# Zhongxu-Wang/ArtSpeech

Measured on AMD Instinct MI355X. Metric: mel frames/sec (whole job; per-GPU = value / n_gpus), acoustic-model inference path, batch 32 x 200-frame utterances, higher is better.
Workload: dtype f32 (f16x3 split-operand MFMA, fp32 accumulate)

## Files before the change

### artspeech_amd/csrc/lstm.hip

```cpp
#include "common.h"
#include "artspeech_hip.h"
#define AS_FILE_CLS AS_CLS_LSTM

#define NB 2

static __device__ __forceinline__ float sigmoidf_(float x) { return __builtin_amdgcn_rcpf(1.0f + __expf(-x)); }
static __device__ __forceinline__ float tanhf_(float x)
{
    const float e = __expf(-2.0f * fabsf(x));
    const float t = (1.0f - e) * __builtin_amdgcn_rcpf(1.0f + e);
    return x < 0.f ? -t : t;
}

template <int CTRL>
static __device__ __forceinline__ float quad_dpp(float v)
{
    return __int_as_float(__builtin_amdgcn_mov_dpp(__float_as_int(v), CTRL, 0xf, 0xf, true));
}

struct LstmJobs { BiLstmJob j[AS_MAX_LSTM_JOBS]; };

static __device__ __forceinline__ void lds_barrier()
{
    asm volatile("s_waitcnt lgkmcnt(0)\n\ts_barrier" ::: "memory");
}

template <int HREG>
__global__ void __launch_bounds__(HREG ? 4 * HREG : 1024)
bilstm_kernel(const LstmJobs jobs, const int* __restrict__ col_off, int B, int Hrt)
{
    extern __shared__ __attribute__((aligned(16))) float sm[];
    const int H = HREG ? HREG : Hrt;
    float* hs = sm;
    float* gs = sm + 2 * H * NB;
    __shared__ int s_off[NB], s_len[NB];

    const BiLstmJob job = jobs.j[blockIdx.z];
    const int dir = blockIdx.y;
    const int u0 = blockIdx.x * NB;
    const int r = threadIdx.x;
    const int G = 4 * H;
    if (r < NB) {
        const int u = u0 + r;
        s_off[r] = u < B ? col_off[u] : 0;
        s_len[r] = u < B ? col_off[u + 1] - col_off[u] : 0;
    }
    for (int i = r; i < 2 * H * NB; i += G) hs[i] = 0.f;
    __syncthreads();
    int Lmax = 0;
#pragma unroll
    for (int u = 0; u < NB; ++u) Lmax = s_len[u] > Lmax ? s_len[u] : Lmax;

    const float* w = job.whh_t + (size_t)dir * H * G + r;
    float wreg[HREG ? HREG : 1];
    if (HREG) {
#pragma unroll
        for (int k = 0; k < HREG; ++k) wreg[k] = w[(size_t)k * G];
    }
    const int unit = r % H, q = r / H;
    float c = 0.f;

    auto load_gx = [&](int t, float (&g)[NB]) {
#pragma unroll
        for (int u = 0; u < NB; ++u) {
            const int L = s_len[u];
            const int pos = dir ? L - 1 - t : t;
            g[u] = (t < L) ? job.gx_tm[(size_t)(s_off[u] + pos) * job.ldg + dir * G + r] : 0.f;
        }
    };
    float gnext[NB];
    load_gx(0, gnext);

    for (int t = 0; t < Lmax; ++t) {
        const float* hc = hs + (t & 1) * H * NB;
        float* hn = hs + ((t + 1) & 1) * H * NB;
        float acc[NB];
#pragma unroll
        for (int u = 0; u < NB; ++u) acc[u] = gnext[u];
        if (t + 1 < Lmax) load_gx(t + 1, gnext);
        if (HREG) {
#pragma unroll
            for (int k = 0; k < HREG; ++k) {
                const float2 h2 = *reinterpret_cast<const float2*>(hc + k * NB);
                acc[0] += wreg[k] * h2.x; acc[1] += wreg[k] * h2.y;
            }
        } else {
            for (int k0 = 0; k0 < H; k0 += 8) {
                float wk[8];
#pragma unroll
                for (int i = 0; i < 8; ++i) wk[i] = w[(size_t)(k0 + i) * G];
#pragma unroll
                for (int i = 0; i < 8; ++i) {
                    const float2 h2 = *reinterpret_cast<const float2*>(hc + (k0 + i) * NB);
                    acc[0] += wk[i] * h2.x; acc[1] += wk[i] * h2.y;
                }
            }
        }
        *reinterpret_cast<float2*>(gs + r * NB) = make_float2(acc[0], acc[1]);
        lds_barrier();
        if (q < NB) {
            const int u = q;
            const int L = s_len[u];
            if (t < L) {
                const float ig = sigmoidf_(gs[(unit)*NB + u]);
                const float fg = sigmoidf_(gs[(H + unit) * NB + u]);
                const float gg = tanhf_(gs[(2 * H + unit) * NB + u]);
                const float og = sigmoidf_(gs[(3 * H + unit) * NB + u]);
                c = fg * c + ig * gg;
                const float hv = og * tanhf_(c);
                hn[unit * NB + u] = hv;
                const int pos = dir ? L - 1 - t : t;
                job.out[(size_t)(dir * H + unit) * job.ldo + s_off[u] + pos] = hv;
            }
        }
        lds_barrier();
    }
}

template <int H, int KREG, int KLDS>
__global__ void __launch_bounds__(2 * H)
bilstm_big_kernel(const LstmJobs jobs, const int* __restrict__ col_off, int B)
{
    constexpr int G = 4 * H, NT = 2 * H, KS = H - KREG - KLDS, SB = 4;
    static_assert(KS >= 0 && KS % SB == 0, "split of the k range");
    extern __shared__ __attribute__((aligned(16))) float sm[];
    float* hs = sm;
    float* gs = hs + 2 * H * NB;
    float* wl = gs + G * NB;
    __shared__ int s_off[NB], s_len[NB];

    const BiLstmJob job = jobs.j[blockIdx.z];
    const int dir = blockIdx.y;
    const int u0 = blockIdx.x * NB;
    const int tid = threadIdx.x;
    if (tid < NB) {
        const int u = u0 + tid;
        s_off[tid] = u < B ? col_off[u] : 0;
        s_len[tid] = u < B ? col_off[u + 1] - col_off[u] : 0;
    }
    for (int i = tid; i < 2 * H * NB; i += NT) hs[i] = 0.f;
    const float* w = job.whh_t + (size_t)dir * H * G + tid;
    float wa[KREG], wb[KREG];
#pragma unroll
    for (int k = 0; k < KREG; ++k) {
        wa[k] = w[(size_t)k * G];
        wb[k] = w[(size_t)k * G + NT];
    }
#pragma unroll 4
    for (int k = 0; k < KLDS; ++k) {
        wl[k * G + tid] = w[(size_t)(KREG + k) * G];
        wl[k * G + NT + tid] = w[(size_t)(KREG + k) * G + NT];
    }
    const float* ws = w + (size_t)(KREG + KLDS) * G;
    __syncthreads();
    int Lmax = 0;
#pragma unroll
    for (int u = 0; u < NB; ++u) Lmax = s_len[u] > Lmax ? s_len[u] : Lmax;
    const int unit = tid % H, q = tid / H;
    float c = 0.f;

    auto load_gx = [&](int t, float (&ga)[NB], float (&gb)[NB]) {
#pragma unroll
        for (int u = 0; u < NB; ++u) {
            const int L = s_len[u];
            const int pos = dir ? L - 1 - t : t;
            const float* p = job.gx_tm + (size_t)(s_off[u] + pos) * job.ldg + dir * G + tid;
            ga[u] = (t < L) ? p[0] : 0.f;
            gb[u] = (t < L) ? p[NT] : 0.f;
        }
    };
    float gna[NB], gnb[NB];
    load_gx(0, gna, gnb);

    for (int t = 0; t < Lmax; ++t) {
        asm volatile("" ::: "memory");
        const float* hc = hs + (t & 1) * H * NB;
        float* hn = hs + ((t + 1) & 1) * H * NB;
        float a0 = gna[0], a1 = gna[1], b0 = gnb[0], b1 = gnb[1];
        if (t + 1 < Lmax) load_gx(t + 1, gna, gnb);
        float ka[SB], kb[SB];
#pragma unroll
        for (int i = 0; i < SB; ++i) {
            ka[i] = ws[(size_t)i * G];
            kb[i] = ws[(size_t)i * G + NT];
        }
#pragma unroll
        for (int k = 0; k < KREG; ++k) {
            const float2 h2 = *reinterpret_cast<const float2*>(hc + k * NB);
            a0 += wa[k] * h2.x; a1 += wa[k] * h2.y;
            b0 += wb[k] * h2.x; b1 += wb[k] * h2.y;
            if ((k & 7) == 7) asm volatile("" ::: "memory");
        }
#pragma unroll 4
        for (int k = 0; k < KLDS; ++k) {
            const float va = wl[k * G + tid], vb = wl[k * G + NT + tid];
            const float2 h2 = *reinterpret_cast<const float2*>(hc + (KREG + k) * NB);
            a0 += va * h2.x; a1 += va * h2.y;
            b0 += vb * h2.x; b1 += vb * h2.y;
        }
        for (int k0 = 0; k0 < KS; k0 += SB) {
            float na[SB], nb[SB];
            const int kn = k0 + SB < KS ? k0 + SB : k0;
#pragma unroll
            for (int i = 0; i < SB; ++i) {
                na[i] = ws[(size_t)(kn + i) * G];
                nb[i] = ws[(size_t)(kn + i) * G + NT];
            }
#pragma unroll
            for (int i = 0; i < SB; ++i) {
                const float2 h2 = *reinterpret_cast<const float2*>(hc + (KREG + KLDS + k0 + i) * NB);
                a0 += ka[i] * h2.x; a1 += ka[i] * h2.y;
                b0 += kb[i] * h2.x; b1 += kb[i] * h2.y;
            }
#pragma unroll
            for (int i = 0; i < SB; ++i) { ka[i] = na[i]; kb[i] = nb[i]; }
        }
        *reinterpret_cast<float2*>(gs + tid * NB) = make_float2(a0, a1);
        *reinterpret_cast<float2*>(gs + (NT + tid) * NB) = make_float2(b0, b1);
        lds_barrier();
        {
            const int u = q;
            const int L = s_len[u];
            if (t < L) {
                const float ig = sigmoidf_(gs[(unit)*NB + u]);
                const float fg = sigmoidf_(gs[(H + unit) * NB + u]);
                const float gg = tanhf_(gs[(2 * H + unit) * NB + u]);
                const float og = sigmoidf_(gs[(3 * H + unit) * NB + u]);
                c = fg * c + ig * gg;
                const float hv = og * tanhf_(c);
                hn[unit * NB + u] = hv;
                const int pos = dir ? L - 1 - t : t;
                job.out[(size_t)(dir * H + unit) * job.ldo + s_off[u] + pos] = hv;
            }
        }
        lds_barrier();
    }
}

template <int H>
__global__ void __launch_bounds__(4 * H)
bilstm_quad_kernel(const LstmJobs jobs, const int* __restrict__ col_off, int B)
{
    constexpr int KQ = H / 4, G = 4 * H;
    __shared__ __attribute__((aligned(16))) float hs[2][H][NB];
    __shared__ int s_off[NB], s_len[NB];
    const BiLstmJob job = jobs.j[blockIdx.z];
    const int dir = blockIdx.y, u0 = blockIdx.x * NB;
    const int tid = threadIdx.x, unit = tid >> 2, kq = tid & 3;
    if (tid < NB) {
        const int u = u0 + tid;
        s_off[tid] = u < B ? col_off[u] : 0;
        s_len[tid] = u < B ? col_off[u + 1] - col_off[u] : 0;
    }
    for (int i = tid; i < 2 * H * NB; i += G) (&hs[0][0][0])[i] = 0.f;
    __syncthreads();
    const int L0 = s_len[0], L1 = s_len[1], o0 = s_off[0], o1 = s_off[1];
    const int Lmax = L0 > L1 ? L0 : L1;

    float w[4][KQ];
    const float* wp = job.whh_t + (size_t)dir * H * G + unit;
#pragma unroll
    for (int g = 0; g < 4; ++g)
#pragma unroll
        for (int kk = 0; kk < KQ; ++kk) w[g][kk] = wp[(size_t)(kq * KQ + kk) * G + g * H];

    const float* gxp = job.gx_tm + dir * G + kq * H + unit;
    auto load_gx = [&](int t, float& g0, float& g1) {
        g0 = (t < L0) ? gxp[(size_t)(o0 + (dir ? L0 - 1 - t : t)) * job.ldg] : 0.f;
        g1 = (t < L1) ? gxp[(size_t)(o1 + (dir ? L1 - 1 - t : t)) * job.ldg] : 0.f;
    };
    constexpr int PF = 4;
    float gq0[PF], gq1[PF];
#pragma unroll
    for (int j = 0; j < PF; ++j) load_gx(j, gq0[j], gq1[j]);
    float c = 0.f;
    const int my_u = kq & 1, my_L = my_u ? L1 : L0, my_o = my_u ? o1 : o0;

    for (int t0 = 0; t0 < Lmax; t0 += PF) {
#pragma unroll
      for (int j = 0; j < PF; ++j) {
        const int t = t0 + j;
        if (t >= Lmax) break;
        const float(*hc)[NB] = hs[t & 1];
        float(*hn)[NB] = hs[(t + 1) & 1];
        float acc[4][2];
#pragma unroll
        for (int g = 0; g < 4; ++g) {
            acc[g][0] = (g == kq) ? gq0[j] : 0.f;
            acc[g][1] = (g == kq) ? gq1[j] : 0.f;
        }
        load_gx(t + PF, gq0[j], gq1[j]);
#pragma unroll
        for (int kk = 0; kk < KQ; ++kk) {
            const float2 h2 = *reinterpret_cast<const float2*>(&hc[kq * KQ + kk][0]);
#pragma unroll
            for (int g = 0; g < 4; ++g) {
                acc[g][0] += w[g][kk] * h2.x;
                acc[g][1] += w[g][kk] * h2.y;
            }
        }
        float pre[4];
#pragma unroll
        for (int g = 0; g < 4; ++g) {
            float a0 = acc[g][0], a1 = acc[g][1];
            a0 += __shfl_xor(a0, 1); a1 += __shfl_xor(a1, 1);
            a0 += __shfl_xor(a0, 2); a1 += __shfl_xor(a1, 2);
            pre[g] = my_u ? a1 : a0;
        }
        if (kq < 2 && t < my_L) {
            const float ig = sigmoidf_(pre[0]), fg = sigmoidf_(pre[1]), gg = tanhf_(pre[2]), og = sigmoidf_(pre[3]);
            c = fg * c + ig * gg;
            const float hv = og * tanhf_(c);
            hn[unit][my_u] = hv;
            job.out[(size_t)(dir * H + unit) * job.ldo + my_o + (dir ? my_L - 1 - t : t)] = hv;
        }
        lds_barrier();
      }
    }
}

typedef float lf2 __attribute__((ext_vector_type(2)));
template <int H>
__global__ void __launch_bounds__(4 * H)
bilstm_quad1_kernel(const LstmJobs jobs, const int* __restrict__ col_off, int B)
{
    constexpr int KQ = H / 4, G = 4 * H;
    static_assert(KQ % 4 == 0, "quarter of the hidden vector in float4 steps");
    __shared__ __attribute__((aligned(16))) float hs[2][H];
    const BiLstmJob job = jobs.j[blockIdx.z];
    const int dir = blockIdx.y, u = blockIdx.x;
    const int tid = threadIdx.x, unit = tid >> 2, kq = tid & 3;
    const int o0 = col_off[u], L = col_off[u + 1] - o0;
    if (L <= 0) return;
    for (int i = tid; i < 2 * H; i += G) (&hs[0][0])[i] = 0.f;
    __syncthreads();

    lf2 wif[KQ], wgo[KQ];
    const float* wp = job.whh_t + (size_t)dir * H * G + unit;
#pragma unroll
    for (int kk = 0; kk < KQ; ++kk) {
        const float* r = wp + (size_t)(kq * KQ + kk) * G;
        wif[kk] = lf2{r[0], r[H]};
        wgo[kk] = lf2{r[2 * H], r[3 * H]};
    }
    const float* gxp = job.gx_tm + dir * G + kq * H + unit;
    auto load_gx = [&](int t) { return (t < L) ? gxp[(size_t)(o0 + (dir ? L - 1 - t : t)) * job.ldg] : 0.f; };
    constexpr int PF = 4;
    float gq[PF];
#pragma unroll
    for (int j = 0; j < PF; ++j) gq[j] = load_gx(j);
    float c = 0.f;
    float* outp = job.out + (size_t)(dir * H + unit) * job.ldo + o0;

    for (int t0 = 0; t0 < L; t0 += PF) {
#pragma unroll
        for (int j = 0; j < PF; ++j) {
            const int t = t0 + j;
            if (t >= L) break;
            const float* hc = hs[t & 1] + kq * KQ;
            float* hn = hs[(t + 1) & 1];
            const float gx = gq[j];
            gq[j] = load_gx(t + PF);
            lf2 aif0 = {0.f, 0.f}, ago0 = {0.f, 0.f}, aif1 = {0.f, 0.f}, ago1 = {0.f, 0.f};
#pragma unroll
            for (int k4 = 0; k4 < KQ; k4 += 4) {
                const float4 h4 = *reinterpret_cast<const float4*>(hc + k4);
                aif0 += wif[k4] * lf2{h4.x, h4.x};
                ago0 += wgo[k4] * lf2{h4.x, h4.x};
                aif1 += wif[k4 + 1] * lf2{h4.y, h4.y};
                ago1 += wgo[k4 + 1] * lf2{h4.y, h4.y};
                aif0 += wif[k4 + 2] * lf2{h4.z, h4.z};
                ago0 += wgo[k4 + 2] * lf2{h4.z, h4.z};
                aif1 += wif[k4 + 3] * lf2{h4.w, h4.w};
                ago1 += wgo[k4 + 3] * lf2{h4.w, h4.w};
            }
            float pre[4] = {aif0[0] + aif1[0], aif0[1] + aif1[1], ago0[0] + ago1[0], ago0[1] + ago1[1]};
#pragma unroll
            for (int g = 0; g < 4; ++g) {
                pre[g] += quad_dpp<0xB1>(pre[g]);
                pre[g] += quad_dpp<0x4E>(pre[g]);
            }
            const float sc = kq == 2 ? 2.f : 1.f;
            const float x = (kq == 0 ? pre[0] : kq == 1 ? pre[1] : kq == 2 ? pre[2] : pre[3]) + gx;
            const float act = fmaf(__builtin_amdgcn_rcpf(1.0f + __expf(-sc * x)), sc, 1.0f - sc);
            const float ig = quad_dpp<0x00>(act), fg = quad_dpp<0x55>(act), gg = quad_dpp<0xAA>(act), og = quad_dpp<0xFF>(act);
            c = fg * c + ig * gg;
            const float hv = og * fmaf(__builtin_amdgcn_rcpf(1.0f + __expf(-2.0f * c)), 2.0f, -1.0f);
            if (kq == 0) {
                hn[unit] = hv;
                outp[dir ? L - 1 - t : t] = hv;
            }
            lds_barrier();
        }
    }
}

extern "C" int as_bilstm_f32(const BiLstmJob* jobs_host, int n_jobs, const int32_t* col_off, int B, int H,
                             as_stream_t stream)
{
    if (!jobs_host || n_jobs <= 0 || n_jobs > AS_MAX_LSTM_JOBS || !col_off || B < 0 || H <= 0 || (4 * H) % 64 ||
        4 * H > 1024 || H % 8)
        return AS_EINVAL;
    LstmJobs jobs;
    for (int i = 0; i < AS_MAX_LSTM_JOBS; ++i) jobs.j[i] = jobs_host[i < n_jobs ? i : 0];
    for (int i = 0; i < n_jobs; ++i)
        if (!jobs.j[i].gx_tm || !jobs.j[i].whh_t || !jobs.j[i].out || jobs.j[i].ldg < 8 * H) return AS_EINVAL;
    if (B == 0) return AS_OK;
    const size_t smem = sizeof(float) * ((size_t)2 * H * NB + (size_t)4 * H * NB);
    const dim3 grid(as_cdiv(B, NB), 2, n_jobs), block(4 * H);
    AsProfScope prof__(AS_FILE_CLS, 0, 0, (hipStream_t)stream);
    const bool single = (H == 64 || H == 128) && (long)n_jobs * 2 * B <= 512;
    if (single) {
        const dim3 g1(B, 2, n_jobs);
        if (H == 64) hipLaunchKernelGGL(bilstm_quad1_kernel<64>, g1, block, 0, (hipStream_t)stream, jobs, col_off, B);
        else hipLaunchKernelGGL(bilstm_quad1_kernel<128>, g1, block, 0, (hipStream_t)stream, jobs, col_off, B);
        AS_CHECK_LAUNCH();
        return AS_OK;
    }
    switch (H) {
    case 16: hipLaunchKernelGGL(bilstm_quad_kernel<16>, grid, block, 0, (hipStream_t)stream, jobs, col_off, B); break;
    case 32: hipLaunchKernelGGL(bilstm_quad_kernel<32>, grid, block, 0, (hipStream_t)stream, jobs, col_off, B); break;
    case 64: hipLaunchKernelGGL(bilstm_quad_kernel<64>, grid, block, 0, (hipStream_t)stream, jobs, col_off, B); break;
    case 128: hipLaunchKernelGGL(bilstm_quad_kernel<128>, grid, block, 0, (hipStream_t)stream, jobs, col_off, B); break;
    case 256: {
        constexpr int KREG = 32, KLDS = 36;
        const size_t sm_big = smem + sizeof(float) * (size_t)KLDS * 1024;
        AS_LDS_OPT_IN((bilstm_big_kernel<256, KREG, KLDS>), (int)sm_big);
        hipLaunchKernelGGL((bilstm_big_kernel<256, KREG, KLDS>), grid, dim3(512), sm_big, (hipStream_t)stream, jobs, col_off, B);
        break;
    }
    default: hipLaunchKernelGGL(bilstm_kernel<0>, grid, block, smem, (hipStream_t)stream, jobs, col_off, B, H); break;
    }
    AS_CHECK_LAUNCH();
    return AS_OK;
}

#define CL_P 4
#define CL_REGION_WORDS 1032
static __device__ __forceinline__ float dpp_add8(float v)
{
    int x = __builtin_bit_cast(int, v);
    v += __builtin_bit_cast(float, __builtin_amdgcn_update_dpp(0, x, 0xB1, 0xF, 0xF, true));
    x = __builtin_bit_cast(int, v);
    v += __builtin_bit_cast(float, __builtin_amdgcn_update_dpp(0, x, 0x4E, 0xF, 0xF, true));
    x = __builtin_bit_cast(int, v);
    v += __builtin_bit_cast(float, __builtin_amdgcn_update_dpp(0, x, 0x141, 0xF, 0xF, true));
    return v;
}

template <int NBU>
__global__ void __launch_bounds__(512)
bilstm_cluster_kernel(const LstmJobs jobs, const int* __restrict__ col_off, int B, int n_clusters, unsigned long long* __restrict__ xchg,
                      unsigned* __restrict__ status, int spin_limit, int drop_member)
{
    constexpr int H = 256, G = 4 * H, UW = H / CL_P, KS = 8, KQ = H / KS, SL = KQ * NBU + 4, HB = KS * SL;
    __shared__ __attribute__((aligned(16))) float hs[2 * HB];
    const int lin = blockIdx.x;
    const int cl = (lin & 7) + 8 * ((lin >> 3) / CL_P), member = (lin >> 3) % CL_P;
    if (cl >= n_clusters) return;
    const int groups = (B + NBU - 1) / NBU;
    const int ug = cl % groups, dir = (cl / groups) & 1;
    const BiLstmJob job = jobs.j[cl / (2 * groups)];
    const int tid = threadIdx.x, ul = tid >> 3, kq = tid & 7, unit = member * UW + ul;
    int off[NBU], len[NBU], Lmax = 0;
#pragma unroll
    for (int i = 0; i < NBU; ++i) {
        const int u = ug * NBU + i;
        off[i] = u < B ? col_off[u] : 0;
        len[i] = u < B ? col_off[u + 1] - col_off[u] : 0;
        Lmax = len[i] > Lmax ? len[i] : Lmax;
    }
    if (Lmax <= 0) return;
    if (member == drop_member) return;
    unsigned long long* region = xchg + (size_t)cl * CL_REGION_WORDS;
    const unsigned epoch = (unsigned)region[0] & 0x7FFFu;
    const unsigned tagbase = epoch << 17;
    unsigned long long* words = region + 1;
    for (int i = tid; i < 2 * HB; i += 512) hs[i] = 0.f;

    lf2 wif[KQ], wgo[KQ];
    const float* wp = job.whh_t + (size_t)dir * H * G + unit;
#pragma unroll
    for (int kk = 0; kk < KQ; ++kk) {
        const float* r = wp + (size_t)(kq * KQ + kk) * G;
        wif[kk] = lf2{r[0], r[H]};
        wgo[kk] = lf2{r[2 * H], r[3 * H]};
    }
    const int gu = kq >> 2, gL = gu < NBU ? len[gu < NBU ? gu : 0] : 0, gO = off[gu < NBU ? gu : 0];
    const float* gxp = job.gx_tm + dir * G + (kq & 3) * H + unit;
    auto load_gx = [&](int t) { return (t < gL) ? gxp[(size_t)(gO + (dir ? gL - 1 - t : t)) * job.ldg] : 0.f; };
    constexpr int PF = 4;
    float gq[PF];
#pragma unroll
    for (int j = 0; j < PF; ++j) gq[j] = load_gx(j);
    float c = 0.f;
    const int my_u = kq < NBU ? kq : 0, my_L = len[my_u], my_o = off[my_u];
    float* outp = job.out + (size_t)(dir * H + unit) * job.ldo + my_o;
    const int pk = tid / NBU, pu = tid % NBU, ppos = (pk / KQ) * SL + (pk % KQ) * NBU + pu;
    __syncthreads();

    for (int t0 = 0; t0 < Lmax; t0 += PF) {
#pragma unroll
        for (int j = 0; j < PF; ++j) {
            const int t = t0 + j;
            if (t >= Lmax) break;
            float* hb = hs + (t & 1) * HB;
            if (t > 0 && tid < H * NBU) {
                const unsigned long long* w = words + (size_t)((t - 1) & 1) * H * NBU + tid;
                const unsigned want = tagbase | (unsigned)t;
                unsigned long long v = __hip_atomic_load(w, __ATOMIC_RELAXED, __HIP_MEMORY_SCOPE_AGENT);
                for (int spin = 0; (unsigned)(v >> 32) != want && spin < spin_limit; ++spin) {
                    __builtin_amdgcn_s_sleep(1);
                    v = __hip_atomic_load(w, __ATOMIC_RELAXED, __HIP_MEMORY_SCOPE_AGENT);
                }
                if ((unsigned)(v >> 32) != want) as_status_raise(status, AS_STATUS_LSTM_TIMEOUT);
                hb[ppos] = __uint_as_float((unsigned)v);
            }
            lds_barrier();
            const float gx = gq[j];
            gq[j] = load_gx(t + PF);
            lf2 aif[NBU], ago[NBU];
#pragma unroll
            for (int u = 0; u < NBU; ++u) {
                aif[u] = lf2{kq == 4 * u ? gx : 0.f, kq == 4 * u + 1 ? gx : 0.f};
                ago[u] = lf2{kq == 4 * u + 2 ? gx : 0.f, kq == 4 * u + 3 ? gx : 0.f};
            }
            const float* hc = hb + kq * SL;
            if (NBU == 2) {
#pragma unroll
                for (int kk = 0; kk < KQ; kk += 2) {
                    const float4 h4 = *reinterpret_cast<const float4*>(hc + kk * 2);
                    aif[0] += wif[kk] * lf2{h4.x, h4.x};
                    ago[0] += wgo[kk] * lf2{h4.x, h4.x};
                    aif[NBU - 1] += wif[kk] * lf2{h4.y, h4.y};
                    ago[NBU - 1] += wgo[kk] * lf2{h4.y, h4.y};
                    aif[0] += wif[kk + 1] * lf2{h4.z, h4.z};
                    ago[0] += wgo[kk + 1] * lf2{h4.z, h4.z};
                    aif[NBU - 1] += wif[kk + 1] * lf2{h4.w, h4.w};
                    ago[NBU - 1] += wgo[kk + 1] * lf2{h4.w, h4.w};
                }
            } else {
                lf2 bif = {0.f, 0.f}, bgo = {0.f, 0.f};
#pragma unroll
                for (int kk = 0; kk < KQ; kk += 4) {
                    const float4 h4 = *reinterpret_cast<const float4*>(hc + kk);
                    aif[0] += wif[kk] * lf2{h4.x, h4.x};
                    ago[0] += wgo[kk] * lf2{h4.x, h4.x};
                    bif += wif[kk + 1] * lf2{h4.y, h4.y};
                    bgo += wgo[kk + 1] * lf2{h4.y, h4.y};
                    aif[0] += wif[kk + 2] * lf2{h4.z, h4.z};
                    ago[0] += wgo[kk + 2] * lf2{h4.z, h4.z};
                    bif += wif[kk + 3] * lf2{h4.w, h4.w};
                    bgo += wgo[kk + 3] * lf2{h4.w, h4.w};
                }
                aif[0] += bif;
                ago[0] += bgo;
            }
            float pre[4] = {0.f, 0.f, 0.f, 0.f};
#pragma unroll
            for (int u = 0; u < NBU; ++u) {
                const float pi = dpp_add8(aif[u][0]), pf = dpp_add8(aif[u][1]), pg = dpp_add8(ago[u][0]), po = dpp_add8(ago[u][1]);
                if (u == my_u) { pre[0] = pi; pre[1] = pf; pre[2] = pg; pre[3] = po; }
            }
            if (kq < NBU) {
                float hv = 0.f;
                if (t < my_L) {
                    const float ig = sigmoidf_(pre[0]), fg = sigmoidf_(pre[1]), gg = tanhf_(pre[2]), og = sigmoidf_(pre[3]);
                    c = fg * c + ig * gg;
                    hv = og * tanhf_(c);
                    outp[dir ? my_L - 1 - t : t] = hv;
                }
                const unsigned long long word = ((unsigned long long)(tagbase | (unsigned)(t + 1)) << 32) | __float_as_uint(hv);
                __hip_atomic_store(words + (size_t)(t & 1) * H * NBU + unit * NBU + kq, word, __ATOMIC_RELAXED, __HIP_MEMORY_SCOPE_AGENT);
            }
        }
    }
    if (member == 0) {
        if (Lmax == 1 && tid < H * NBU) {
            const unsigned long long* w = words + tid;
            const unsigned want = tagbase | 1u;
            unsigned long long v = __hip_atomic_load(w, __ATOMIC_RELAXED, __HIP_MEMORY_SCOPE_AGENT);
            for (int spin = 0; (unsigned)(v >> 32) != want && spin < spin_limit; ++spin) {
                __builtin_amdgcn_s_sleep(1);
                v = __hip_atomic_load(w, __ATOMIC_RELAXED, __HIP_MEMORY_SCOPE_AGENT);
            }
            if ((unsigned)(v >> 32) != want) as_status_raise(status, AS_STATUS_LSTM_TIMEOUT);
        }
        __syncthreads();
        if (tid == 0) region[0] = epoch + 1;
    }
}

static int g_cl_drop_member = -1, g_cl_spin_limit = 1 << 21;
extern "C" int as_bilstm_cluster_test_hooks(int drop_member, int spin_limit)
{
    if (drop_member < -1 || drop_member >= CL_P || spin_limit < 0) return AS_EINVAL;
    g_cl_drop_member = drop_member;
    g_cl_spin_limit = spin_limit > 0 ? spin_limit : 1 << 21;
    return AS_OK;
}

extern "C" size_t as_bilstm_cluster_bytes(int n_jobs, int B)
{
    if (n_jobs <= 0 || B <= 0) return 0;
    return (size_t)n_jobs * 2 * B * CL_REGION_WORDS * sizeof(unsigned long long);
}

extern "C" int as_bilstm_cluster_f32(const BiLstmJob* jobs_host, int n_jobs, const int32_t* col_off, int B, int H, int max_len, void* xchg,
                                     size_t xchg_bytes, as_stream_t stream)
{
    if (!jobs_host || n_jobs <= 0 || n_jobs > AS_MAX_LSTM_JOBS || !col_off || B < 0 || H <= 0) return AS_EINVAL;
    if (B == 0) return AS_OK;
    const long c1 = (long)n_jobs * 2 * B, c2 = (long)n_jobs * 2 * ((B + 1) / 2);
    const int nbu = c1 * CL_P <= 256 ? 1 : (c2 * CL_P <= 256 ? 2 : 0);
    const char* mode = getenv("AS_LSTM_CLUSTER");
    const int use = mode ? atoi(mode) : nbu;
    if (H != 256 || !xchg || use <= 0 || use > 2 || max_len <= 0 || max_len >= (1 << 17) || (use == 1 ? c1 : c2) * CL_P > 256 ||
        xchg_bytes < as_bilstm_cluster_bytes(n_jobs, B))
        return as_bilstm_f32(jobs_host, n_jobs, col_off, B, H, stream);
    LstmJobs jobs;
    for (int i = 0; i < AS_MAX_LSTM_JOBS; ++i) jobs.j[i] = jobs_host[i < n_jobs ? i : 0];
    for (int i = 0; i < n_jobs; ++i)
        if (!jobs.j[i].gx_tm || !jobs.j[i].whh_t || !jobs.j[i].out || jobs.j[i].ldg < 8 * H) return AS_EINVAL;
    const int ncl = (int)(use == 1 ? c1 : c2);
    const dim3 grid(8 * CL_P * as_cdiv(ncl, 8)), block(512);
    unsigned* status = as_status_words_device();
    AsProfScope prof__(AS_FILE_CLS, 0, 0, (hipStream_t)stream);
    if (use == 1)
        hipLaunchKernelGGL(bilstm_cluster_kernel<1>, grid, block, 0, (hipStream_t)stream, jobs, col_off, B, ncl,
                           static_cast<unsigned long long*>(xchg), status, g_cl_spin_limit, g_cl_drop_member);
    else
        hipLaunchKernelGGL(bilstm_cluster_kernel<2>, grid, block, 0, (hipStream_t)stream, jobs, col_off, B, ncl,
                           static_cast<unsigned long long*>(xchg), status, g_cl_spin_limit, g_cl_drop_member);
    AS_CHECK_LAUNCH();
    return AS_OK;
}
```

Measured before the change: 1.730 million.

## Pack multiple utterances per LSTM block sized to device CU count

Adds a bilstm_quadn kernel in which each block steps NU utterances (2 or 4) together. The recurrent weights held in registers are reused across those utterances, and one LDS barrier per timestep is shared among them. The host picks NU from the CU count so that the grid roughly fills the device, replacing the fixed threshold of 512 blocks that decided between the single-utterance kernel and the NB-batched one. The cost is that utterances of unequal length in one block run to the longest of them, plus extra register pressure from the per-utterance prefetch arrays.

```diff
diff --git a/artspeech_amd/csrc/lstm.hip b/artspeech_amd/csrc/lstm.hip
--- a/artspeech_amd/csrc/lstm.hip
+++ b/artspeech_amd/csrc/lstm.hip
@@ -320,6 +320,38 @@
 }
 
 typedef float lf2 __attribute__((ext_vector_type(2)));
+template <int KQ>
+static __device__ __forceinline__ float quad_cell_step(const lf2 (&wif)[KQ], const lf2 (&wgo)[KQ], const float* hc, float gx, int kq,
+                                                       float c, float& c_new)
+{
+    lf2 aif0 = {0.f, 0.f}, ago0 = {0.f, 0.f}, aif1 = {0.f, 0.f}, ago1 = {0.f, 0.f};
+#pragma unroll
+    for (int k4 = 0; k4 < KQ; k4 += 4) {
+        const float4 h4 = *reinterpret_cast<const float4*>(hc + k4);
+        aif0 += wif[k4] * lf2{h4.x, h4.x};
+        ago0 += wgo[k4] * lf2{h4.x, h4.x};
+        aif1 += wif[k4 + 1] * lf2{h4.y, h4.y};
+        ago1 += wgo[k4 + 1] * lf2{h4.y, h4.y};
+        aif0 += wif[k4 + 2] * lf2{h4.z, h4.z};
+        ago0 += wgo[k4 + 2] * lf2{h4.z, h4.z};
+        aif1 += wif[k4 + 3] * lf2{h4.w, h4.w};
+        ago1 += wgo[k4 + 3] * lf2{h4.w, h4.w};
+    }
+    float pre[4] = {aif0[0] + aif1[0], aif0[1] + aif1[1], ago0[0] + ago1[0], ago0[1] + ago1[1]};
+#pragma unroll
+    for (int g = 0; g < 4; ++g) {
+        pre[g] += quad_dpp<0xB1>(pre[g]);
+        pre[g] += quad_dpp<0x4E>(pre[g]);
+    }
+    const float sc = kq == 2 ? 2.f : 1.f;
+    const float p01 = kq & 1 ? pre[1] : pre[0], p23 = kq & 1 ? pre[3] : pre[2];
+    const float x = (kq & 2 ? p23 : p01) + gx;
+    const float act = fmaf(__builtin_amdgcn_rcpf(1.0f + __expf(-sc * x)), sc, 1.0f - sc);
+    const float ig = quad_dpp<0x00>(act), fg = quad_dpp<0x55>(act), gg = quad_dpp<0xAA>(act), og = quad_dpp<0xFF>(act);
+    c_new = fmaf(fg, c, ig * gg);
+    return og * fmaf(__builtin_amdgcn_rcpf(1.0f + __expf(-2.0f * c_new)), 2.0f, -1.0f);
+}
+
 template <int H>
 __global__ void __launch_bounds__(4 * H)
 bilstm_quad1_kernel(const LstmJobs jobs, const int* __restrict__ col_off, int B)
@@ -357,35 +389,10 @@
         for (int j = 0; j < PF; ++j) {
             const int t = t0 + j;
             if (t >= L) break;
-            const float* hc = hs[t & 1] + kq * KQ;
             float* hn = hs[(t + 1) & 1];
             const float gx = gq[j];
             gq[j] = load_gx(t + PF);
-            lf2 aif0 = {0.f, 0.f}, ago0 = {0.f, 0.f}, aif1 = {0.f, 0.f}, ago1 = {0.f, 0.f};
-#pragma unroll
-            for (int k4 = 0; k4 < KQ; k4 += 4) {
-                const float4 h4 = *reinterpret_cast<const float4*>(hc + k4);
-                aif0 += wif[k4] * lf2{h4.x, h4.x};
-                ago0 += wgo[k4] * lf2{h4.x, h4.x};
-                aif1 += wif[k4 + 1] * lf2{h4.y, h4.y};
-                ago1 += wgo[k4 + 1] * lf2{h4.y, h4.y};
-                aif0 += wif[k4 + 2] * lf2{h4.z, h4.z};
-                ago0 += wgo[k4 + 2] * lf2{h4.z, h4.z};
-                aif1 += wif[k4 + 3] * lf2{h4.w, h4.w};
-                ago1 += wgo[k4 + 3] * lf2{h4.w, h4.w};
-            }
-            float pre[4] = {aif0[0] + aif1[0], aif0[1] + aif1[1], ago0[0] + ago1[0], ago0[1] + ago1[1]};
-#pragma unroll
-            for (int g = 0; g < 4; ++g) {
-                pre[g] += quad_dpp<0xB1>(pre[g]);
-                pre[g] += quad_dpp<0x4E>(pre[g]);
-            }
-            const float sc = kq == 2 ? 2.f : 1.f;
-            const float x = (kq == 0 ? pre[0] : kq == 1 ? pre[1] : kq == 2 ? pre[2] : pre[3]) + gx;
-            const float act = fmaf(__builtin_amdgcn_rcpf(1.0f + __expf(-sc * x)), sc, 1.0f - sc);
-            const float ig = quad_dpp<0x00>(act), fg = quad_dpp<0x55>(act), gg = quad_dpp<0xAA>(act), og = quad_dpp<0xFF>(act);
-            c = fg * c + ig * gg;
-            const float hv = og * fmaf(__builtin_amdgcn_rcpf(1.0f + __expf(-2.0f * c)), 2.0f, -1.0f);
+            const float hv = quad_cell_step<KQ>(wif, wgo, hs[t & 1] + kq * KQ, gx, kq, c, c);
             if (kq == 0) {
                 hn[unit] = hv;
                 outp[dir ? L - 1 - t : t] = hv;
@@ -393,6 +400,106 @@
             lds_barrier();
         }
     }
+}
+
+template <int H, int NU>
+__global__ void __launch_bounds__(4 * H)
+bilstm_quadn_kernel(const LstmJobs jobs, const int* __restrict__ col_off, int B)
+{
+    constexpr int KQ = H / 4, G = 4 * H, PF = 4;
+    static_assert(KQ % 4 == 0, "quarter of the hidden vector in float4 steps");
+    __shared__ __attribute__((aligned(16))) float hs[2][NU][H];
+    const BiLstmJob job = jobs.j[blockIdx.z];
+    const int dir = blockIdx.y, u0 = blockIdx.x * NU;
+    const int tid = threadIdx.x, unit = tid >> 2, kq = tid & 3;
+    const int last_row = col_off[B] - 1;
+    int off[NU], len[NU], safe[NU], Lmax = 0;
+#pragma unroll
+    for (int i = 0; i < NU; ++i) {
+        const int u = u0 + i < B ? u0 + i : B - 1;
+        off[i] = col_off[u];
+        len[i] = u0 + i < B ? col_off[u + 1] - off[i] : 0;
+        safe[i] = off[i] < last_row ? off[i] : last_row;
+        Lmax = len[i] > Lmax ? len[i] : Lmax;
+    }
+    if (Lmax <= 0) return;
+    for (int i = tid; i < 2 * NU * H; i += G) (&hs[0][0][0])[i] = 0.f;
+    __syncthreads();
+
+    lf2 wif[KQ], wgo[KQ];
+    const float* wp = job.whh_t + (size_t)dir * H * G + unit;
+#pragma unroll
+    for (int kk = 0; kk < KQ; ++kk) {
+        const float* r = wp + (size_t)(kq * KQ + kk) * G;
+        wif[kk] = lf2{r[0], r[H]};
+        wgo[kk] = lf2{r[2 * H], r[3 * H]};
+    }
+    const float* gxp = job.gx_tm + dir * G + kq * H + unit;
+    auto load_gx = [&](int i, int t) {
+        const int row = t < len[i] ? off[i] + (dir ? len[i] - 1 - t : t) : safe[i];
+        return gxp[(size_t)row * job.ldg];
+    };
+    float gq[NU][PF], c[NU];
+#pragma unroll
+    for (int j = 0; j < PF; ++j)
+#pragma unroll
+        for (int i = 0; i < NU; ++i) gq[i][j] = load_gx(i, j);
+#pragma unroll
+    for (int i = 0; i < NU; ++i) c[i] = 0.f;
+    float* outp = job.out + (size_t)(dir * H + unit) * job.ldo;
+    __builtin_amdgcn_s_waitcnt(0x0F70);
+
+    for (int t0 = 0; t0 < Lmax; t0 += PF) {
+#pragma unroll
+        for (int j = 0; j < PF; ++j) {
+            const int t = t0 + j;
+            float gx[NU];
+#pragma unroll
+            for (int i = 0; i < NU; ++i) {
+                gx[i] = t < len[i] ? gq[i][j] : 0.f;
+                asm volatile("" : "+v"(gx[i]) : : "memory");
+            }
+#pragma unroll
+            for (int i = 0; i < NU; ++i) gq[i][j] = load_gx(i, t + PF);
+#pragma unroll
+            for (int i = 0; i < NU; ++i) {
+                float cn;
+                const float hv = quad_cell_step<KQ>(wif, wgo, hs[t & 1][i] + kq * KQ, gx[i], kq, c[i], cn);
+                const bool live = t < len[i];
+                c[i] = live ? cn : c[i];
+                if (kq == 0 && live) {
+                    hs[(t + 1) & 1][i][unit] = hv;
+                    outp[off[i] + (dir ? len[i] - 1 - t : t)] = hv;
+                }
+            }
+            lds_barrier();
+        }
+    }
+}
+
+static int device_cu_count(int* cus)
+{
+    static int cache[64];
+    int d = 0;
+    AS_CHECK(hipGetDevice(&d));
+    int n = __atomic_load_n(&cache[d & 63], __ATOMIC_RELAXED);
+    if (n <= 0) {
+        hipDeviceProp_t prop;
+        AS_CHECK(hipGetDeviceProperties(&prop, d));
+        n = prop.multiProcessorCount;
+        if (n <= 0) return AS_EINVAL;
+        __atomic_store_n(&cache[d & 63], n, __ATOMIC_RELAXED);
+    }
+    *cus = n;
+    return AS_OK;
+}
+
+template <int H>
+static void launch_quad_group(int nu, dim3 grid, dim3 block, hipStream_t stream, const LstmJobs& jobs, const int* col_off, int B)
+{
+    if (nu == 1) hipLaunchKernelGGL(bilstm_quad1_kernel<H>, grid, block, 0, stream, jobs, col_off, B);
+    else if (nu == 2) hipLaunchKernelGGL((bilstm_quadn_kernel<H, 2>), grid, block, 0, stream, jobs, col_off, B);
+    else hipLaunchKernelGGL((bilstm_quadn_kernel<H, 4>), grid, block, 0, stream, jobs, col_off, B);
 }
 
 extern "C" int as_bilstm_f32(const BiLstmJob* jobs_host, int n_jobs, const int32_t* col_off, int B, int H,
@@ -408,12 +515,18 @@
     if (B == 0) return AS_OK;
     const size_t smem = sizeof(float) * ((size_t)2 * H * NB + (size_t)4 * H * NB);
     const dim3 grid(as_cdiv(B, NB), 2, n_jobs), block(4 * H);
+    int nu = 0;
+    if (H == 64 || H == 128) {
+        int cus = 0;
+        const int rc = device_cu_count(&cus);
+        if (rc != AS_OK) return rc;
+        for (nu = 1; nu <= 4 && (long)n_jobs * 2 * as_cdiv(B, nu) > cus; nu *= 2) {}
+    }
     AsProfScope prof__(AS_FILE_CLS, 0, 0, (hipStream_t)stream);
-    const bool single = (H == 64 || H == 128) && (long)n_jobs * 2 * B <= 512;
-    if (single) {
-        const dim3 g1(B, 2, n_jobs);
-        if (H == 64) hipLaunchKernelGGL(bilstm_quad1_kernel<64>, g1, block, 0, (hipStream_t)stream, jobs, col_off, B);
-        else hipLaunchKernelGGL(bilstm_quad1_kernel<128>, g1, block, 0, (hipStream_t)stream, jobs, col_off, B);
+    if (nu >= 1 && nu <= 4) {
+        const dim3 gn(as_cdiv(B, nu), 2, n_jobs);
+        if (H == 64) launch_quad_group<64>(nu, gn, block, (hipStream_t)stream, jobs, col_off, B);
+        else launch_quad_group<128>(nu, gn, block, (hipStream_t)stream, jobs, col_off, B);
         AS_CHECK_LAUNCH();
         return AS_OK;
     }
```

Result: no change. 1.739 million, median of 6 (+0.5%).
